# maxsonate/video-diffusion-nnx

Hardware: AMD Instinct MI355X
Metric: denoised frames/sec, 16fx64x64 1000-step DDPM (higher is better)
Workload: dtype bf16; 1 GPU; config_v2_2 (north-star shape): Unet3D dim=64 C=1, 16f x 64x64, DDPM T=1000 p_sample_loop (UNet forward + p_sample per step, hipGraph replay); value = n_gpus*B*F/(T*s_per_step); batch_per_gpu=64, parallelism=dp1 (independent samples, no collective), mfma_operands=bf16, storage=weights fp32 master, activations bf16, fp32 accumulate, process_group=none (single process)

## Files before the change

### video_diffusion_nnx_amd/csrc/conv_pw.hip

```cpp
#include "vdx_common.h"
#include "vdx_internal.h"

namespace vdx {

typedef unsigned pu32x4 __attribute__((ext_vector_type(4)));

template <int ROWS, int KS = 4, bool OUT32 = false>
__global__ __launch_bounds__(512) void conv1x1_pw_kernel(const ConvArgs P, const int nct, const int groups_per_range, const int ngroups) {
    using M = Mma<MODE_BF16>;
    constexpr int TM = ROWS / 16, TN = 2;
    constexpr int KBB = KS * 64;
    extern __shared__ __attribute__((aligned(16))) char smem[];
    const int Cin = P.C0 + P.C1, nkb = Cin / (32 * KS);
    const int WRS = Cin * 2 + 16;
    char* Wl = smem;
    float* bl = reinterpret_cast<float*>(Wl + ROWS * WRS);

    const int tid = threadIdx.x, lane = tid & 63, wave = tid >> 6, lp = lane & 15, q = lane >> 4;
    const int ct = (blockIdx.x >> 3) % nct, range = ((blockIdx.x >> 3) / nct) * 8 + (blockIdx.x & 7);
    const int co0 = ct * ROWS;
    const int g0 = range * groups_per_range, g1 = min(g0 + groups_per_range, ngroups);
    if (g0 >= g1) return;

    {
        const int cpr = Cin >> 3;
        const char* wsrc = reinterpret_cast<const char*>(P.wp);
        for (int i = tid; i < ROWS * cpr; i += 512) {
            const int row = i / cpr, c = i - row * cpr;
            const int tm = row >> 4, rr = row & 15;
            const int co = co0 + (tm >> 1) * 32 + (rr >> 2) * 8 + (tm & 1) * 4 + (rr & 3);
            *reinterpret_cast<uint4*>(Wl + row * WRS + c * 16) = *reinterpret_cast<const uint4*>(wsrc + ((size_t)(P.wrow0 + co) * P.CinPad + c * 8) * 2);
        }
        for (int i = tid; i < ROWS; i += 512) bl[i] = P.bias ? P.bias[co0 + i] : 0.f;
    }
    __syncthreads();

    const __amdgpu_buffer_rsrc_t rx0 = __builtin_amdgcn_make_buffer_rsrc(const_cast<float*>(P.x0), 0, P.x0_bytes, 0x00020000);
    const __amdgpu_buffer_rsrc_t rx1 = __builtin_amdgcn_make_buffer_rsrc(const_cast<float*>(P.C1 ? P.x1 : P.x0), 0, P.C1 ? P.x1_bytes : P.x0_bytes, 0x00020000);
    const int nkb0 = P.C0 / (32 * KS);
    const unsigned rb0 = P.C0 * 2, rb1 = P.C1 * 2;

    auto load_block = [&](int g, int kb, pu32x4 (&xf)[KS][TN]) {
        const bool second = kb >= nkb0;
        const unsigned rb = second ? rb1 : rb0;
        const unsigned base = (unsigned)(g * 32 + lp) * rb + (unsigned)((second ? kb - nkb0 : kb) * KBB + q * 16);
#pragma unroll
        for (int s = 0; s < KS; ++s)
#pragma unroll
            for (int tn = 0; tn < TN; ++tn) {
                const unsigned off = base + tn * 16 * rb + s * 64;
                xf[s][tn] = second ? __builtin_amdgcn_raw_buffer_load_b128(rx1, off, 0, 0) : __builtin_amdgcn_raw_buffer_load_b128(rx0, off, 0, 0);
            }
    };
    f32x4 acc[TM][TN];
    auto mma_block = [&](int kb, const pu32x4 (&xf)[KS][TN]) {
#pragma unroll
        for (int s = 0; s < KS; ++s) {
            uint4 bf[TN];
#pragma unroll
            for (int tn = 0; tn < TN; ++tn) bf[tn] = make_uint4(xf[s][tn].x, xf[s][tn].y, xf[s][tn].z, xf[s][tn].w);
#pragma unroll
            for (int tm = 0; tm < TM; ++tm) {
                const uint4 af = *reinterpret_cast<const uint4*>(Wl + (tm * 16 + lp) * WRS + kb * KBB + s * 64 + q * 16);
#pragma unroll
                for (int tn = 0; tn < TN; ++tn) M::mma(acc[tm][tn], af, bf[tn]);
            }
        }
    };

    char* const yb = reinterpret_cast<char*>(P.y);
    const char* const resb = reinterpret_cast<const char*>(P.res);
    constexpr bool PP = ROWS == 64 && KS == 4;
    auto init_acc = [&]() {
#pragma unroll
        for (int tm = 0; tm < TM; ++tm) {
            const float4 b4 = *reinterpret_cast<const float4*>(bl + (tm >> 1) * 32 + q * 8 + (tm & 1) * 4);
#pragma unroll
            for (int tn = 0; tn < TN; ++tn) acc[tm][tn] = f32x4{b4.x, b4.y, b4.z, b4.w};
        }
    };
    auto store_group = [&](int g) {
#pragma unroll
        for (int tn = 0; tn < TN; ++tn) {
            const size_t pix = (size_t)g * 32 + tn * 16 + lp;
#pragma unroll
            for (int j = 0; j < TM / 2; ++j) {
                const size_t el = pix * P.Cout + co0 + j * 32 + q * 8;
                float o[8];
#pragma unroll
                for (int k = 0; k < 4; ++k) { o[k] = acc[2 * j][tn][k]; o[4 + k] = acc[2 * j + 1][tn][k]; }
                if constexpr (OUT32) {
                    if (resb) {
                        const float4 r0 = *reinterpret_cast<const float4*>(resb + el * 4), r1 = *reinterpret_cast<const float4*>(resb + el * 4 + 16);
                        o[0] += r0.x; o[1] += r0.y; o[2] += r0.z; o[3] += r0.w; o[4] += r1.x; o[5] += r1.y; o[6] += r1.z; o[7] += r1.w;
                    }
                    *reinterpret_cast<float4*>(yb + el * 4) = make_float4(o[0], o[1], o[2], o[3]);
                    *reinterpret_cast<float4*>(yb + el * 4 + 16) = make_float4(o[4], o[5], o[6], o[7]);
                } else {
                    const size_t e = el * 2;
                    if (resb) {
                        const uint4 r = *reinterpret_cast<const uint4*>(resb + e);
                        o[0] += __uint_as_float(r.x << 16); o[1] += __uint_as_float(r.x & 0xFFFF0000u);
                        o[2] += __uint_as_float(r.y << 16); o[3] += __uint_as_float(r.y & 0xFFFF0000u);
                        o[4] += __uint_as_float(r.z << 16); o[5] += __uint_as_float(r.z & 0xFFFF0000u);
                        o[6] += __uint_as_float(r.w << 16); o[7] += __uint_as_float(r.w & 0xFFFF0000u);
                    }
                    *reinterpret_cast<uint4*>(yb + e) = make_uint4(pack_bf16x2(o[0], o[1]), pack_bf16x2(o[2], o[3]), pack_bf16x2(o[4], o[5]), pack_bf16x2(o[6], o[7]));
                }
            }
        }
    };
    if constexpr (KS == 2) {
        pu32x4 xa[KS][TN], xb[KS][TN];
        int g = g0 + wave;
        if (g < g1) load_block(g, 0, xa);
        for (; g < g1; g += 16) {
            __asm__ volatile("" ::: "memory");
            if (g + 8 < g1) load_block(g + 8, 0, xb);
            init_acc(); mma_block(0, xa); store_group(g);
            if (g + 8 >= g1) break;
            if (g + 16 < g1) load_block(g + 16, 0, xa);
            init_acc(); mma_block(0, xb); store_group(g + 8);
        }
    } else {
        pu32x4 xa[KS][TN], xb[PP ? KS : 1][TN];
        for (int g = g0 + wave; g < g1; g += 8) {
            __asm__ volatile("" ::: "memory");
            init_acc();
            load_block(g, 0, xa);
            if constexpr (PP) {
                for (int kb = 0; kb < nkb; kb += 2) {
                    if (kb + 1 < nkb) load_block(g, kb + 1, xb);
                    mma_block(kb, xa);
                    if (kb + 1 >= nkb) break;
                    if (kb + 2 < nkb) load_block(g, kb + 2, xa);
                    mma_block(kb + 1, xb);
                }
            } else {
                for (int kb = 0; kb < nkb; ++kb) {
                    mma_block(kb, xa);
                    if (kb + 1 < nkb) load_block(g, kb + 1, xa);
                }
            }
            store_group(g);
        }
    }
}

int conv1x1_pw_rows(const ConvArgs& a) {
    const int cin = a.C0 + a.C1;
    if (a.Cout % 128 == 0 && (size_t)128 * (cin * 2 + 16) + 128 * 4 <= 140 * 1024) return 128;
    return 64;
}

bool conv1x1_pw_eligible(int mode, const ConvArgs& a) {
    if (mode != MODE_BF16 || a.kind != 0 || a.kh != 1 || a.kw != 1 || a.stride != 1 || a.pad != 0 || a.pro || a.out_stats) return false;
    if (!a.x0_bf16 || (a.C1 && !a.x1_bf16)) return false;
    const bool out32 = !a.y_bf16;
    if (a.res && (a.res_bf16 != 0) == out32) return false;
    const int cin = a.C0 + a.C1;
    if ((cin % 128 && cin != 64) || cin > 1024 || a.Cout % 64 || a.Cout < 64) return false;
    if (out32 && cin == 64) return false;
    if (!out32 && cin != 64 && a.Cout < 128) return false;
    if (a.C1 && (a.C0 % 128 || a.C1 % 128)) return false;
    if (a.CinPad != cin) return false;
    const size_t npix = (size_t)a.NF * a.H * a.W;
    if (npix % 32 || npix < 32 * 256) return false;
    if (npix * (size_t)std::max(std::max(a.C0, a.C1), a.Cout) * 2 >= 0xFFFF0000ull) return false;
    const int rows = conv1x1_pw_rows(a);
    if ((size_t)rows * (cin * 2 + 16) + rows * 4 > 160 * 1024) return false;
    return true;
}

hipError_t launch_conv1x1_pw(const ConvArgs& a, hipStream_t st) {
    const int cin = a.C0 + a.C1, rows = conv1x1_pw_rows(a), nct = a.Cout / rows;
    const int ngroups = (int)((size_t)a.NF * a.H * a.W / 32);
    const int cus = device_cus();
    const size_t lds = (size_t)rows * (cin * 2 + 16) + rows * 4;
    const int wg_per_cu = (lds <= 80 * 1024 && rows == 128) ? 2 : 1;
    int nranges = std::max(8, (cus * wg_per_cu / nct) / 8 * 8);
    int gpr = ((ngroups + nranges - 1) / nranges + 7) / 8 * 8;
    nranges = ((ngroups + gpr - 1) / gpr + 7) / 8 * 8;
    auto go = [&](auto kfn) -> hipError_t {
        if (hipError_t e = lds_opt_in(kfn, lds); e != hipSuccess) return e;
        hipLaunchKernelGGL(kfn, dim3(nranges * nct), dim3(512), lds, st, a, nct, gpr, ngroups);
        return hipGetLastError();
    };
    if (!a.y_bf16) return rows == 128 ? go(conv1x1_pw_kernel<128, 4, true>) : go(conv1x1_pw_kernel<64, 4, true>);
    if (cin == 64) return rows == 128 ? go(conv1x1_pw_kernel<128, 2>) : go(conv1x1_pw_kernel<64, 2>);
    return rows == 128 ? go(conv1x1_pw_kernel<128>) : go(conv1x1_pw_kernel<64>);
}

}
```

### video_diffusion_nnx_amd/csrc/elementwise.hip

```cpp
#include "vdx_common.h"
#include <stdlib.h>
#include "vdx_internal.h"

namespace vdx {

template <int VPL>
__global__ __launch_bounds__(256) void resblock_tail_kernel(TailArgs P) {
    __shared__ float coefA[1024], coefD[1024];
    __shared__ float gm[64];
    const int tid = threadIdx.x;
    const int C = P.C;
    const int b = blockIdx.y;
    gn_mean_rstd_wg(P.stats, b, P.groups, (double)P.pix_per_sample * (C / P.groups), gm, tid, 256);
    __syncthreads();
    for (int c = tid; c < C; c += 256) {
        const int g = c / (C / P.groups);
        const float a = gm[2 * g + 1] * P.gn_gamma[c];
        coefA[c] = a;
        coefD[c] = P.gn_beta[c] - gm[2 * g] * a;
    }
    __syncthreads();
    const int LPP = P.lpp;
    const int ppb = 256 / LPP;
    const int sub = tid % LPP, pl = tid / LPP;
    const float invC = 1.0f / (float)C;
    for (long pix = (long)blockIdx.x * ppb + pl; pix < P.pix_per_sample; pix += (long)gridDim.x * ppb) {
        const size_t base = ((size_t)b * P.pix_per_sample + pix) * C;
        float4 r[VPL];
        float s = 0.f, ss = 0.f;
#pragma unroll
        for (int v = 0; v < VPL; ++v) {
            const int c = (v * LPP + sub) * 4;
            r[v] = make_float4(0.f, 0.f, 0.f, 0.f);
            if (c < C) {
                r[v] = load4_f32_or_bf16(P.r, base + c, P.r_bf16);
                s += r[v].x + r[v].y + r[v].z + r[v].w;
                ss += r[v].x * r[v].x + r[v].y * r[v].y + r[v].z * r[v].z + r[v].w * r[v].w;
            }
        }
        for (int o = 1; o < LPP; o <<= 1) { s += __shfl_xor(s, o); ss += __shfl_xor(ss, o); }
        const float mean = s * invC;
        const float var = fmaxf(ss * invC - mean * mean, 0.f);
        const float rstd = rsqrtf(var + NORM_EPS);
#pragma unroll
        for (int v = 0; v < VPL; ++v) {
            const int c = (v * LPP + sub) * 4;
            if (c < C) {
                const float4 y = load4_f32_or_bf16(P.y2, base + c, P.y2_bf16);
                const float4 a = *reinterpret_cast<const float4*>(coefA + c);
                const float4 d = *reinterpret_cast<const float4*>(coefD + c);
                const float4 lg = *reinterpret_cast<const float4*>(P.ln_gamma + c);
                const float4 lb = *reinterpret_cast<const float4*>(P.ln_beta + c);
                float4 o;
                o.x = silu_f(fmaf(y.x, a.x, d.x)) + fmaf((r[v].x - mean) * rstd, lg.x, lb.x);
                o.y = silu_f(fmaf(y.y, a.y, d.y)) + fmaf((r[v].y - mean) * rstd, lg.y, lb.y);
                o.z = silu_f(fmaf(y.z, a.z, d.z)) + fmaf((r[v].z - mean) * rstd, lg.z, lb.z);
                o.w = silu_f(fmaf(y.w, a.w, d.w)) + fmaf((r[v].w - mean) * rstd, lg.w, lb.w);
                store4_f32_or_bf16(P.out, base + c, o, P.out_bf16);
            }
        }
    }
}

__device__ __forceinline__ void unpack8(const uint4& u, float (&f)[8]) {
    f[0] = __uint_as_float(u.x << 16); f[1] = __uint_as_float(u.x & 0xFFFF0000u);
    f[2] = __uint_as_float(u.y << 16); f[3] = __uint_as_float(u.y & 0xFFFF0000u);
    f[4] = __uint_as_float(u.z << 16); f[5] = __uint_as_float(u.z & 0xFFFF0000u);
    f[6] = __uint_as_float(u.w << 16); f[7] = __uint_as_float(u.w & 0xFFFF0000u);
}

template <int VPL>
__global__ __launch_bounds__(256) void resblock_tail16_kernel(TailArgs P) {
    __shared__ float coefA[1024], coefD[1024];
    __shared__ float gm[64];
    const int tid = threadIdx.x;
    const int C = P.C;
    const int b = blockIdx.y;
    gn_mean_rstd_wg(P.stats, b, P.groups, (double)P.pix_per_sample * (C / P.groups), gm, tid, 256);
    __syncthreads();
    for (int c = tid; c < C; c += 256) {
        const int g = c / (C / P.groups);
        const float a = gm[2 * g + 1] * P.gn_gamma[c];
        coefA[c] = a;
        coefD[c] = P.gn_beta[c] - gm[2 * g] * a;
    }
    __syncthreads();
    const int LPP = P.lpp;
    const int ppb = 256 / LPP;
    const int sub = tid % LPP, pl = tid / LPP;
    const float invC = 1.0f / (float)C;
    const char* rb = reinterpret_cast<const char*>(P.r);
    const char* yb = reinterpret_cast<const char*>(P.y2);
    char* ob = reinterpret_cast<char*>(P.out);
    for (long pix = (long)blockIdx.x * ppb + pl; pix < P.pix_per_sample; pix += (long)gridDim.x * ppb) {
        const size_t base = ((size_t)b * P.pix_per_sample + pix) * C;
        float r[VPL][8];
        float s = 0.f, ss = 0.f;
#pragma unroll
        for (int v = 0; v < VPL; ++v) {
            const int c = (v * LPP + sub) * 8;
#pragma unroll
            for (int k = 0; k < 8; ++k) r[v][k] = 0.f;
            if (c < C) {
                unpack8(*reinterpret_cast<const uint4*>(rb + (base + c) * 2), r[v]);
#pragma unroll
                for (int k = 0; k < 8; ++k) { s += r[v][k]; ss += r[v][k] * r[v][k]; }
            }
        }
        for (int o = 1; o < LPP; o <<= 1) { s += __shfl_xor(s, o); ss += __shfl_xor(ss, o); }
        const float mean = s * invC;
        const float var = fmaxf(ss * invC - mean * mean, 0.f);
        const float rstd = rsqrtf(var + NORM_EPS);
#pragma unroll
        for (int v = 0; v < VPL; ++v) {
            const int c = (v * LPP + sub) * 8;
            if (c < C) {
                float y[8], o[8];
                unpack8(*reinterpret_cast<const uint4*>(yb + (base + c) * 2), y);
#pragma unroll
                for (int k = 0; k < 8; ++k)
                    o[k] = silu_f(fmaf(y[k], coefA[c + k], coefD[c + k])) + fmaf((r[v][k] - mean) * rstd, P.ln_gamma[c + k], P.ln_beta[c + k]);
                *reinterpret_cast<uint4*>(ob + (base + c) * 2) =
                    make_uint4(pack_bf16x2(o[0], o[1]), pack_bf16x2(o[2], o[3]), pack_bf16x2(o[4], o[5]), pack_bf16x2(o[6], o[7]));
            }
        }
    }
}

__global__ __launch_bounds__(256) void gn_silu_apply16_kernel(unsigned* __restrict__ y, const double* __restrict__ stats, const float* __restrict__ gamma,
                                                              const float* __restrict__ beta, const float* __restrict__ ss, int ss_stride, int groups,
                                                              int C, long pix_per_sample) {
    __shared__ float coefA[1024], coefD[1024];
    __shared__ float gm[64];
    const int tid = threadIdx.x, b = blockIdx.y;
    gn_mean_rstd_wg(stats, b, groups, (double)pix_per_sample * (C / groups), gm, tid, 256);
    __syncthreads();
    for (int c = tid; c < C; c += 256) {
        const int g = c / (C / groups);
        const float m = gm[2 * g], rs = gm[2 * g + 1];
        const float ga = gamma[c], be = beta[c];
        float sc = 1.f, sh = 0.f;
        if (ss) { sc = ss[(size_t)b * ss_stride + c] + 1.f; sh = ss[(size_t)b * ss_stride + C + c]; }
        coefA[c] = rs * ga * sc;
        coefD[c] = (be - m * rs * ga) * sc + sh;
    }
    __syncthreads();
    const int octs = C >> 3;
    const long n = pix_per_sample * octs;
    uint4* base = reinterpret_cast<uint4*>(y) + (size_t)b * n;
    for (long i0 = (long)blockIdx.x * 1024 + tid; i0 < n; i0 += (long)gridDim.x * 1024) {
        uint4 v[4];
#pragma unroll
        for (int u = 0; u < 4; ++u) v[u] = (i0 + u * 256 < n) ? base[i0 + u * 256] : make_uint4(0u, 0u, 0u, 0u);
#pragma unroll
        for (int u = 0; u < 4; ++u) {
            if (i0 + u * 256 >= n) continue;
            const int c = (int)((i0 + u * 256) % octs) * 8;
            float f[8], o[8];
            unpack8(v[u], f);
#pragma unroll
            for (int k = 0; k < 8; ++k) o[k] = silu_f(fmaf(f[k], coefA[c + k], coefD[c + k]));
            base[i0 + u * 256] = make_uint4(pack_bf16x2(o[0], o[1]), pack_bf16x2(o[2], o[3]), pack_bf16x2(o[4], o[5]), pack_bf16x2(o[6], o[7]));
        }
    }
}

hipError_t launch_gn_silu_apply16(float* y_bf16, const double* stats, const float* gamma, const float* beta, const float* ss, int ss_stride, int groups,
                                  int C, int batch, long pix_per_sample, hipStream_t st) {
    if (C % 8 || C > 1024 || groups <= 0 || groups > 32 || C % groups) return hipErrorInvalidValue;
    const long n = pix_per_sample * (C / 8);
    const int gx = (int)std::max<long>(1, std::min<long>((n + 1023) / 1024, 2048));
    LaunchScope ls(st, "gn_silu_apply16_kernel", 8.0 * batch * pix_per_sample * C, 4.0 * batch * pix_per_sample * C, "C%d px%ld x %d", C, pix_per_sample, batch);
    hipLaunchKernelGGL(gn_silu_apply16_kernel, dim3(gx, batch), dim3(256), 0, st, reinterpret_cast<unsigned*>(y_bf16), stats, gamma, beta, ss, ss_stride, groups, C, pix_per_sample);
    return hipGetLastError();
}

typedef unsigned tu32x4 __attribute__((ext_vector_type(4)));

template <int CIN, int COUT, bool CAT, bool FIN = false>
__global__ __launch_bounds__(256, (CIN == 128 && COUT == 64) ? 4 : (COUT <= 128 ? 3 : 2)) void resblock_tail_rc16_kernel(TailArgs P) {
    using M = Mma<MODE_BF16>;
    constexpr int NTM = COUT / 16, NKS = CIN / 32, NH = COUT / 32;
    constexpr int C0 = CAT ? CIN / 2 : CIN, NK0 = C0 / 32;
    constexpr int WRS = CIN * 2 + 16;
    extern __shared__ __attribute__((aligned(16))) char smem[];
    char* Wl = smem;
    float* coefA = reinterpret_cast<float*>(Wl + COUT * WRS);
    float* coefD = coefA + COUT;
    float* lng = coefD + COUT;
    float* lnb = lng + COUT;
    float* rcb = lnb + COUT;
    float* gm = rcb + COUT;
    float* finw = gm + 64;
    const int tid = threadIdx.x, lane = tid & 63, wave = tid >> 6, lp = lane & 15, q = lane >> 4;
    const int b = blockIdx.y;
    for (int i = tid; i < COUT * (CIN / 8); i += 256) {
        const int row = i / (CIN / 8), c = i % (CIN / 8);
        const int tm = row >> 4, rr = row & 15;
        const int co = (tm >> 1) * 32 + (rr >> 2) * 8 + (tm & 1) * 4 + (rr & 3);
        *reinterpret_cast<uint4*>(Wl + row * WRS + c * 16) =
            *reinterpret_cast<const uint4*>(reinterpret_cast<const char*>(P.rc_w) + ((size_t)co * ((CIN + 63) / 64 * 64) + c * 8) * 2);
    }
    gn_mean_rstd_wg(P.stats, b, P.groups, (double)P.pix_per_sample * (COUT / P.groups), gm, tid, 256);
    __syncthreads();
    for (int c = tid; c < COUT; c += 256) {
        const int g = c / (COUT / P.groups);
        const float a = gm[2 * g + 1] * P.gn_gamma[c];
        coefA[c] = a;
        coefD[c] = P.gn_beta[c] - gm[2 * g] * a;
        lng[c] = P.ln_gamma[c]; lnb[c] = P.ln_beta[c]; rcb[c] = P.rc_b[c];
        if (FIN) finw[c] = P.fin_w[c];
    }
    __syncthreads();

    const unsigned pps = (unsigned)P.pix_per_sample;
    const char* x0p = reinterpret_cast<const char*>(P.x0) + (size_t)b * pps * C0 * 2;
    const char* x1p = CAT ? reinterpret_cast<const char*>(P.x1) + (size_t)b * pps * C0 * 2 : x0p;
    const char* y2p = reinterpret_cast<const char*>(P.y2) + (size_t)b * pps * COUT * 2;
    char* outp = FIN ? const_cast<char*>(y2p) : reinterpret_cast<char*>(P.out) + (size_t)b * pps * COUT * 2;
    float* const finp = FIN ? P.fin_out + (size_t)b * pps : nullptr;
    const float finb = FIN ? P.fin_b[0] : 0.f;
    const __amdgpu_buffer_rsrc_t rx0 = __builtin_amdgcn_make_buffer_rsrc(const_cast<char*>(x0p), 0, pps * C0 * 2, 0x00020000);
    const __amdgpu_buffer_rsrc_t rx1 = __builtin_amdgcn_make_buffer_rsrc(const_cast<char*>(x1p), 0, pps * C0 * 2, 0x00020000);
    const __amdgpu_buffer_rsrc_t ry = __builtin_amdgcn_make_buffer_rsrc(const_cast<char*>(y2p), 0, pps * COUT * 2, 0x00020000);
    const __amdgpu_buffer_rsrc_t ro = __builtin_amdgcn_make_buffer_rsrc(outp, 0, pps * COUT * 2, 0x00020000);
    const int ngroups = (int)(pps >> 4);
    const int gstride = (int)gridDim.x * 4;
    const unsigned lane_x = lp * (C0 * 2) + q * 16, lane_y = lp * (COUT * 2) + q * 16;

    auto issue = [&](int g, tu32x4 (&xf)[NKS], tu32x4 (&yf)[NH]) {
        const unsigned ox = (unsigned)g * (16 * C0 * 2) + lane_x, oy = (unsigned)g * (16 * COUT * 2) + lane_y;
#pragma unroll
        for (int s = 0; s < NKS; ++s)
            xf[s] = (s < NK0) ? __builtin_amdgcn_raw_buffer_load_b128(rx0, ox + s * 64, 0, 0)
                              : __builtin_amdgcn_raw_buffer_load_b128(rx1, ox + (s - NK0) * 64, 0, 0);
#pragma unroll
        for (int j = 0; j < NH; ++j) yf[j] = __builtin_amdgcn_raw_buffer_load_b128(ry, oy + j * 64, 0, 0);
    };
    auto compute = [&](int g, const tu32x4 (&xf)[NKS], const tu32x4 (&yf)[NH]) {
        __asm__ volatile("" ::: "memory");
        f32x4 acc[NTM];
#pragma unroll
        for (int tm = 0; tm < NTM; ++tm) {
            const float4 b4 = *reinterpret_cast<const float4*>(rcb + (tm >> 1) * 32 + q * 8 + (tm & 1) * 4);
            acc[tm] = f32x4{b4.x, b4.y, b4.z, b4.w};
        }
#pragma unroll
        for (int s = 0; s < NKS; ++s) {
            const uint4 bx = make_uint4(xf[s].x, xf[s].y, xf[s].z, xf[s].w);
#pragma unroll
            for (int tm = 0; tm < NTM; ++tm)
                M::mma(acc[tm], *reinterpret_cast<const uint4*>(Wl + (tm * 16 + lp) * WRS + s * 64 + q * 16), bx);
        }
        float s1 = 0.f, s2 = 0.f;
#pragma unroll
        for (int tm = 0; tm < NTM; ++tm)
#pragma unroll
            for (int e = 0; e < 4; ++e) { s1 += acc[tm][e]; s2 += acc[tm][e] * acc[tm][e]; }
        s1 = reduce_q(s1); s2 = reduce_q(s2);
        const float mean = s1 * (1.0f / COUT);
        const float var = fmaxf(s2 * (1.0f / COUT) - mean * mean, 0.f);
        const float rstd = rsqrtf(var + NORM_EPS);
        const unsigned oy = (unsigned)g * (16 * COUT * 2) + lane_y;
        float dot = 0.f;
#pragma unroll
        for (int j = 0; j < NH; ++j) {
            float y[8], o[8];
            unpack8(make_uint4(yf[j].x, yf[j].y, yf[j].z, yf[j].w), y);
            const int c0 = j * 32 + q * 8;
#pragma unroll
            for (int h = 0; h < 2; ++h) {
                const float4 a4 = *reinterpret_cast<const float4*>(coefA + c0 + 4 * h), d4 = *reinterpret_cast<const float4*>(coefD + c0 + 4 * h);
                const float4 g4 = *reinterpret_cast<const float4*>(lng + c0 + 4 * h), e4 = *reinterpret_cast<const float4*>(lnb + c0 + 4 * h);
                const f32x4 r = acc[2 * j + h];
                o[4 * h + 0] = silu_f(fmaf(y[4 * h + 0], a4.x, d4.x)) + fmaf((r[0] - mean) * rstd, g4.x, e4.x);
                o[4 * h + 1] = silu_f(fmaf(y[4 * h + 1], a4.y, d4.y)) + fmaf((r[1] - mean) * rstd, g4.y, e4.y);
                o[4 * h + 2] = silu_f(fmaf(y[4 * h + 2], a4.z, d4.z)) + fmaf((r[2] - mean) * rstd, g4.z, e4.z);
                o[4 * h + 3] = silu_f(fmaf(y[4 * h + 3], a4.w, d4.w)) + fmaf((r[3] - mean) * rstd, g4.w, e4.w);
            }
            if constexpr (FIN) {
                const float4 w0 = *reinterpret_cast<const float4*>(finw + c0), w1 = *reinterpret_cast<const float4*>(finw + c0 + 4);
                dot = fmaf(o[0], w0.x, dot); dot = fmaf(o[1], w0.y, dot); dot = fmaf(o[2], w0.z, dot); dot = fmaf(o[3], w0.w, dot);
                dot = fmaf(o[4], w1.x, dot); dot = fmaf(o[5], w1.y, dot); dot = fmaf(o[6], w1.z, dot); dot = fmaf(o[7], w1.w, dot);
            } else {
                __builtin_amdgcn_raw_buffer_store_b128(tu32x4{pack_bf16x2(o[0], o[1]), pack_bf16x2(o[2], o[3]), pack_bf16x2(o[4], o[5]), pack_bf16x2(o[6], o[7])},
                                                       ro, oy + j * 64, 0, 0);
            }
        }
        if constexpr (FIN) {
            dot = reduce_q(dot);
            if (q == 0) finp[(size_t)g * 16 + lp] = dot + finb;
        }
    };

    tu32x4 xa[NKS], ya[NH], xb[NKS], yb[NH];
    int g = (int)blockIdx.x * 4 + wave;
    if (g < ngroups) issue(g, xa, ya);
    while (g < ngroups) {
        const int g1 = g + gstride;
        if (g1 < ngroups) issue(g1, xb, yb);
        compute(g, xa, ya);
        if (g1 >= ngroups) break;
        g = g1 + gstride;
        if (g < ngroups) issue(g, xa, ya);
        compute(g1, xb, yb);
    }
}

bool tail_rc16_supported(int cin, int c0, int cout, long pix_per_sample) {
    const bool shape = (cin == 128 && cout == 64) || (cin == 64 && cout == 128) || (cin == 256 && cout == 64) || (cin == 128 && cout == 256) ||
                       (cin == 64 && cout == 32) || (cin == 32 && cout == 64) || (cin == 128 && cout == 32);
    return shape && (c0 == cin || 2 * c0 == cin) && pix_per_sample % 16 == 0 && pix_per_sample * std::max(cin, cout) * 2 < (1L << 31);
}

template <int CIN, int COUT>
static hipError_t launch_tail_rc16(const TailArgs& a, hipStream_t st) {
    const size_t lds = (size_t)COUT * (CIN * 2 + 16) + (6 * COUT + 64) * sizeof(float);
    const long need = (a.pix_per_sample / 16 + 3) / 4;
    const long gx = std::min<long>(need, std::max<long>(std::max<long>(1, need / 8), (2048 + a.batch - 1) / std::max(1, a.batch)));
    auto go = [&](auto kfn) -> hipError_t {
        if (hipError_t e = lds_opt_in(kfn, lds); e != hipSuccess) return e;
        const double px = (double)a.batch * a.pix_per_sample;
        LaunchScope ls(st, "resblock_tail_rc16_kernel", 2.0 * px * CIN * COUT + (a.fin_w ? 2.0 * px * COUT : 0.0),
                       px * (CIN + (a.fin_w ? 1.0 : 2.0) * COUT) * 2 + (a.fin_w ? px * 4 : 0.0) + 2.0 * CIN * COUT, "<%d, %d, %s> px%ld x %d", CIN, COUT,
                       a.fin_w ? "true, head" : (a.C1 ? "true" : "false"), a.pix_per_sample, a.batch);
        hipLaunchKernelGGL(kfn, dim3((unsigned)gx, a.batch), dim3(256), lds, st, a);
        return hipGetLastError();
    };
    if constexpr ((CIN == 128 && COUT == 64) || (CIN == 64 && COUT == 32)) {
        if (a.fin_w) return a.C1 ? go(resblock_tail_rc16_kernel<CIN, COUT, true, true>) : hipErrorInvalidValue;
    } else if (a.fin_w) return hipErrorInvalidValue;
    return a.C1 ? go(resblock_tail_rc16_kernel<CIN, COUT, true>) : go(resblock_tail_rc16_kernel<CIN, COUT, false>);
}

hipError_t launch_resblock_tail(TailArgs a, hipStream_t st) {
    if (a.rc_w) {
        const int cin = a.C0 + a.C1;
        if (!(a.y2_bf16 && a.out_bf16) || !a.x0 || (a.C1 && !a.x1) || !a.rc_b || !tail_rc16_supported(cin, a.C0, a.C, a.pix_per_sample))
            return hipErrorInvalidValue;
        if (a.groups <= 0 || a.groups > 32 || a.C % a.groups) return hipErrorInvalidValue;
        if (cin == 128 && a.C == 64) return launch_tail_rc16<128, 64>(a, st);
        if (cin == 64 && a.C == 128) return launch_tail_rc16<64, 128>(a, st);
        if (cin == 256 && a.C == 64) return launch_tail_rc16<256, 64>(a, st);
        if (cin == 64 && a.C == 32) return launch_tail_rc16<64, 32>(a, st);
        if (cin == 32 && a.C == 64) return launch_tail_rc16<32, 64>(a, st);
        if (cin == 128 && a.C == 32) return launch_tail_rc16<128, 32>(a, st);
        return launch_tail_rc16<128, 256>(a, st);
    }
    if (a.y2_bf16 && a.r_bf16 && a.out_bf16 && a.C % 8 == 0) {
        const int octs = a.C / 8;
        int lpp = 1;
        while (lpp < octs && lpp < 64) lpp <<= 1;
        a.lpp = lpp;
        const int vpl = (octs + lpp - 1) / lpp;
        const int ppb = 256 / lpp;
        const int tail_wgs = 0;
        const long need = (a.pix_per_sample + ppb - 1) / ppb;
        const long total = tail_wgs > 0 ? tail_wgs : std::max<long>(2048, need * a.batch / 8);
        const int gx = (int)std::min<long>(need, std::max<long>(1, std::min<long>(2048, total / std::max(1, a.batch))));
        dim3 grid(gx, a.batch);
        const double el = (double)a.batch * a.pix_per_sample * a.C;
        LaunchScope ls(st, "resblock_tail16_kernel", 10.0 * el, 3.0 * el * 2, "<%d> C%d px%ld x %d", vpl, a.C, a.pix_per_sample, a.batch);
        switch (vpl) {
            case 1: hipLaunchKernelGGL(resblock_tail16_kernel<1>, grid, dim3(256), 0, st, a); break;
            case 2: hipLaunchKernelGGL(resblock_tail16_kernel<2>, grid, dim3(256), 0, st, a); break;
            default: return hipErrorInvalidValue;
        }
        return hipGetLastError();
    }
    const int quads = a.C / 4;
    int lpp = 1;
    while (lpp < quads && lpp < 64) lpp <<= 1;
    a.lpp = lpp;
    const int vpl = (quads + lpp - 1) / lpp;
    const int ppb = 256 / lpp;
    const int tail_wgs32 = 0;
    const long need32 = (a.pix_per_sample + ppb - 1) / ppb;
    const long total32 = tail_wgs32 > 0 ? tail_wgs32 : std::max<long>(2048, need32 * a.batch / 8);
    int gx = (int)std::min<long>(need32, std::max<long>(1, std::min<long>(2048, total32 / std::max(1, a.batch))));
    dim3 grid(gx, a.batch);
    const double el = (double)a.batch * a.pix_per_sample * a.C;
    LaunchScope ls(st, "resblock_tail_kernel", 10.0 * el, el * ((a.y2_bf16 ? 2.0 : 4.0) + (a.r_bf16 ? 2.0 : 4.0) + (a.out_bf16 ? 2.0 : 4.0)), "<%d> C%d px%ld x %d y2_16 %d", vpl == 3 ? 4 : vpl,
                   a.C, a.pix_per_sample, a.batch, a.y2_bf16);
    switch (vpl) {
        case 1: hipLaunchKernelGGL(resblock_tail_kernel<1>, grid, dim3(256), 0, st, a); break;
        case 2: hipLaunchKernelGGL(resblock_tail_kernel<2>, grid, dim3(256), 0, st, a); break;
        case 3: case 4: hipLaunchKernelGGL(resblock_tail_kernel<4>, grid, dim3(256), 0, st, a); break;
        default: return hipErrorInvalidValue;
    }
    return hipGetLastError();
}

__global__ __launch_bounds__(256) void init_conv_kernel(const float* __restrict__ x, const float* __restrict__ w,
                                                        const float* __restrict__ bias, float* __restrict__ y,
                                                        int B, int Cin, int F, int H, int W, int Cout, int K, int y_bf16) {
    extern __shared__ float tile[];
    const int pad = K / 2, TW = 16 + K - 1;
    const int tx = blockIdx.x % ((W + 15) / 16), ty = blockIdx.x / ((W + 15) / 16);
    const int f = blockIdx.y % F, b = blockIdx.y / F;
    const int cg = blockIdx.z;
    for (int i = threadIdx.x; i < Cin * TW * TW; i += 256) {
        const int c = i / (TW * TW), r = i % (TW * TW);
        const int gy = ty * 16 + r / TW - pad, gx = tx * 16 + r % TW - pad;
        float v = 0.f;
        if (gy >= 0 && gy < H && gx >= 0 && gx < W) v = x[((((size_t)b * Cin + c) * F + f) * H + gy) * W + gx];
        tile[i] = v;
    }
    __syncthreads();
    const int px = threadIdx.x & 15, py = threadIdx.x >> 4;
    float acc[16];
#pragma unroll
    for (int j = 0; j < 16; ++j) acc[j] = 0.f;
    const int co0 = cg * 16;
    for (int c = 0; c < Cin; ++c)
        for (int ky = 0; ky < K; ++ky)
            for (int kx = 0; kx < K; ++kx) {
                const float v = tile[(c * TW + py + ky) * TW + px + kx];
                const float* wr = w + ((size_t)(ky * K + kx) * Cin + c) * Cout + co0;
#pragma unroll
                for (int j = 0; j < 16; ++j) acc[j] = fmaf(v, (co0 + j < Cout) ? wr[j] : 0.f, acc[j]);
            }
    const int oy = ty * 16 + py, ox = tx * 16 + px;
    if (oy < H && ox < W) {
        const size_t ob = ((((size_t)b * F + f) * H + oy) * W + ox) * Cout + co0;
        if (co0 + 16 <= Cout) {
#pragma unroll
            for (int j = 0; j < 16; j += 4)
                store4_f32_or_bf16(y, ob + j, make_float4(acc[j] + bias[co0 + j], acc[j + 1] + bias[co0 + j + 1],
                                                          acc[j + 2] + bias[co0 + j + 2], acc[j + 3] + bias[co0 + j + 3]), y_bf16);
        } else {
            for (int j = 0; j < 16 && co0 + j < Cout; ++j) {
                if (y_bf16) reinterpret_cast<__bf16*>(y)[ob + j] = (__bf16)(acc[j] + bias[co0 + j]);
                else y[ob + j] = acc[j] + bias[co0 + j];
            }
        }
    }
}

__global__ __launch_bounds__(256) void init_conv_mfma_kernel(const float* __restrict__ x, const float* __restrict__ w,
                                                             const float* __restrict__ bias, float* __restrict__ y,
                                                             int B, int F, int H, int W, int Cout, int K, int y_bf16) {
    using M = Mma<MODE_BF16>;
    constexpr int KP = 64, RSK = KP * 2 + 16;
    constexpr int TWM = 16 + 8 - 1;
    extern __shared__ __attribute__((aligned(16))) char smem[];
    float* tile = reinterpret_cast<float*>(smem);
    char* wl = smem + ((TWM * TWM * 4 + 15) / 16) * 16;
    char* col = wl + 64 * RSK;
    const int tid = threadIdx.x, lane = tid & 63, wv = tid >> 6;
    const int lp = lane & 15, q = lane >> 4;
    const int pad = K / 2, TW = 16 + K - 1;
    const int tx = blockIdx.x % ((W + 15) / 16), ty = blockIdx.x / ((W + 15) / 16);
    const int f = blockIdx.y % F, b = blockIdx.y / F;
    for (int i = tid; i < TW * TW; i += 256) {
        const int gy = ty * 16 + i / TW - pad, gx = tx * 16 + i % TW - pad;
        tile[i] = (gy >= 0 && gy < H && gx >= 0 && gx < W) ? x[(((size_t)b * F + f) * H + gy) * W + gx] : 0.f;
    }
    for (int i = tid; i < 64 * RSK / 4; i += 256) reinterpret_cast<unsigned*>(wl)[i] = 0u;
    __syncthreads();
    {
        float wr[16];
        const int nw = K * K * Cout;
#pragma unroll
        for (int u = 0; u < 16; ++u) { const int i = tid + u * 256; wr[u] = w[i < nw ? i : 0]; }
#pragma unroll
        for (int u = 0; u < 16; ++u) {
            const int i = tid + u * 256;
            if (i < nw) {
                const int co = i % Cout, t = i / Cout;
                if (co < 64) M::store1(wl + co * RSK, (t / K) * 8 + (t % K), wr[u]);
            }
        }
    }
    {
        const int py = tid >> 4, px = tid & 15;
        char* row = col + tid * RSK;
#pragma unroll
        for (int ky = 0; ky < 8; ++ky) {
            float v[8];
#pragma unroll
            for (int kx = 0; kx < 8; ++kx) v[kx] = (ky < K && kx < K) ? tile[(py + ky) * TW + px + kx] : 0.f;
            *reinterpret_cast<uint4*>(row + ky * 16) =
                make_uint4(pack_bf16x2(v[0], v[1]), pack_bf16x2(v[2], v[3]), pack_bf16x2(v[4], v[5]), pack_bf16x2(v[6], v[7]));
        }
    }
    __syncthreads();
    f32x4 acc[4][4];
#pragma unroll
    for (int i = 0; i < 4; ++i)
#pragma unroll
        for (int j = 0; j < 4; ++j) acc[i][j] = f32x4{0.f, 0.f, 0.f, 0.f};
#pragma unroll
    for (int ch = 0; ch < 2; ++ch) {
        uint4 af[4], bf[4];
#pragma unroll
        for (int tm = 0; tm < 4; ++tm) af[tm] = *reinterpret_cast<const uint4*>(wl + (tm * 16 + lp) * RSK + ch * 64 + q * 16);
#pragma unroll
        for (int tn = 0; tn < 4; ++tn) bf[tn] = *reinterpret_cast<const uint4*>(col + ((wv * 4 + tn) * 16 + lp) * RSK + ch * 64 + q * 16);
#pragma unroll
        for (int tm = 0; tm < 4; ++tm)
#pragma unroll
            for (int tn = 0; tn < 4; ++tn) M::mma(acc[tm][tn], af[tm], bf[tn]);
    }
    if (y_bf16 && Cout == 64) {
        __syncthreads();
#pragma unroll
        for (int tn = 0; tn < 4; ++tn)
#pragma unroll
            for (int tm = 0; tm < 4; ++tm) {
                const float4 bi = *reinterpret_cast<const float4*>(bias + tm * 16 + 4 * q);
                *reinterpret_cast<uint2*>(col + ((wv * 4 + tn) * 16 + lp) * RSK + (tm * 16 + 4 * q) * 2) =
                    make_uint2(pack_bf16x2(acc[tm][tn][0] + bi.x, acc[tm][tn][1] + bi.y), pack_bf16x2(acc[tm][tn][2] + bi.z, acc[tm][tn][3] + bi.w));
            }
        __syncthreads();
#pragma unroll
        for (int u = 0; u < 8; ++u) {
            const int i = tid + u * 256, p = i >> 3, pc = i & 7;
            const int oy = ty * 16 + (p >> 4), ox = tx * 16 + (p & 15);
            if (oy < H && ox < W)
                *reinterpret_cast<uint4*>(reinterpret_cast<char*>(y) + (((((size_t)b * F + f) * H + oy) * W + ox) * 64) * 2 + pc * 16) =
                    *reinterpret_cast<const uint4*>(col + p * RSK + pc * 16);
        }
        return;
    }
#pragma unroll
    for (int tn = 0; tn < 4; ++tn) {
        const int p = (wv * 4 + tn) * 16 + lp;
        const int oy = ty * 16 + (p >> 4), ox = tx * 16 + (p & 15);
        if (oy >= H || ox >= W) continue;
        const size_t ob = ((((size_t)b * F + f) * H + oy) * W + ox) * Cout;
#pragma unroll
        for (int tm = 0; tm < 4; ++tm) {
            const int co = tm * 16 + 4 * q;
            if (co >= Cout) continue;
            const float4 bi = *reinterpret_cast<const float4*>(bias + co);
            store4_f32_or_bf16(y, ob + co, make_float4(acc[tm][tn][0] + bi.x, acc[tm][tn][1] + bi.y, acc[tm][tn][2] + bi.z, acc[tm][tn][3] + bi.w), y_bf16);
        }
    }
}

hipError_t launch_init_conv(const float* x, const float* w, const float* bias, float* y, int B, int Cin, int F, int H, int W,
                            int Cout, int K, int y_bf16, hipStream_t st) {
    return launch_init_conv_mode(MODE_F32, x, w, bias, y, B, Cin, F, H, W, Cout, K, y_bf16, st);
}

hipError_t launch_init_conv_mode(int mode, const float* x, const float* w, const float* bias, float* y, int B, int Cin, int F, int H, int W,
                                 int Cout, int K, int y_bf16, hipStream_t st) {
    if (mode == MODE_BF16 && Cin == 1 && K <= 8 && Cout <= 64 && Cout % 4 == 0) {
        const size_t lds = ((23 * 23 * 4 + 15) / 16) * 16 + (size_t)(64 + 256) * (64 * 2 + 16);
        dim3 grid(((W + 15) / 16) * ((H + 15) / 16), B * F);
        const double px = (double)B * F * H * W;
        LaunchScope ls(st, "init_conv_mfma_kernel", 2.0 * px * K * K * Cout, px * (4.0 + Cout * (y_bf16 ? 2.0 : 4.0)), "k%d 1->%d %dx%dx%d", K, Cout, B * F, H, W);
        hipLaunchKernelGGL(init_conv_mfma_kernel, grid, dim3(256), lds, st, x, w, bias, y, B, F, H, W, Cout, K, y_bf16);
        return hipGetLastError();
    }
    const int TW = 16 + K - 1;
    dim3 grid(((W + 15) / 16) * ((H + 15) / 16), B * F, (Cout + 15) / 16);
    const double px = (double)B * F * H * W;
    LaunchScope ls(st, "init_conv_kernel", 2.0 * px * K * K * Cin * Cout, px * (4.0 * Cin + Cout * (y_bf16 ? 2.0 : 4.0)), "k%d %d->%d %dx%dx%d", K, Cin, Cout, B * F, H, W);
    hipLaunchKernelGGL(init_conv_kernel, grid, dim3(256), (size_t)Cin * TW * TW * 4, st, x, w, bias, y, B, Cin, F, H, W, Cout, K, y_bf16);
    return hipGetLastError();
}

__global__ __launch_bounds__(256) void final_conv_kernel(const float* __restrict__ x, const float* __restrict__ w,
                                                         const float* __restrict__ bias, float* __restrict__ y,
                                                         long npix, int D, int Cout, int lpp, int x_bf16) {
    const int sub = threadIdx.x % lpp, pl = threadIdx.x / lpp, ppb = 256 / lpp;
    for (long pix = (long)blockIdx.x * ppb + pl; pix < npix; pix += (long)gridDim.x * ppb) {
        for (int co = 0; co < Cout; ++co) {
            float s = 0.f;
            if (x_bf16) {
                for (int c = sub * 8; c < D; c += lpp * 8) {
                    float v[8];
                    unpack8(*reinterpret_cast<const uint4*>(reinterpret_cast<const char*>(x) + ((size_t)pix * D + c) * 2), v);
#pragma unroll
                    for (int k = 0; k < 8; ++k) s = fmaf(v[k], w[(size_t)(c + k) * Cout + co], s);
                }
            } else {
                for (int c = sub * 4; c < D; c += lpp * 4) {
                    const float4 v = *reinterpret_cast<const float4*>(x + (size_t)pix * D + c);
                    s += v.x * w[(size_t)c * Cout + co] + v.y * w[(size_t)(c + 1) * Cout + co]
                       + v.z * w[(size_t)(c + 2) * Cout + co] + v.w * w[(size_t)(c + 3) * Cout + co];
                }
            }
            for (int o = 1; o < lpp; o <<= 1) s += __shfl_xor(s, o);
            if (sub == 0) y[(size_t)pix * Cout + co] = s + bias[co];
        }
    }
}

template <int COUT>
__global__ __launch_bounds__(256) void final_conv16_kernel(const float* __restrict__ x, const float* __restrict__ w,
                                                           const float* __restrict__ bias, float* __restrict__ y, long npix, int D, int lpp) {
    constexpr int U = 4;
    const int sub = threadIdx.x % lpp, pl = threadIdx.x / lpp, ppb = 256 / lpp;
    float wr[COUT][8], br[COUT];
#pragma unroll
    for (int co = 0; co < COUT; ++co) {
        br[co] = bias[co];
#pragma unroll
        for (int k = 0; k < 8; ++k) wr[co][k] = w[(size_t)(sub * 8 + k) * COUT + co];
    }
    for (long g0 = (long)blockIdx.x * U; g0 * ppb < npix; g0 += (long)gridDim.x * U) {
        uint4 raw[U];
#pragma unroll
        for (int u = 0; u < U; ++u) {
            const long pix = (g0 + u) * ppb + pl;
            raw[u] = *reinterpret_cast<const uint4*>(reinterpret_cast<const char*>(x) + ((size_t)(pix < npix ? pix : 0) * D + sub * 8) * 2);
        }
#pragma unroll
        for (int u = 0; u < U; ++u) {
            const long pix = (g0 + u) * ppb + pl;
            float v[8];
            unpack8(raw[u], v);
#pragma unroll
            for (int co = 0; co < COUT; ++co) {
                float s = 0.f;
#pragma unroll
                for (int k = 0; k < 8; ++k) s = fmaf(v[k], wr[co][k], s);
                for (int o = 1; o < lpp; o <<= 1) s += __shfl_xor(s, o);
                if (sub == 0 && pix < npix) y[(size_t)pix * COUT + co] = s + br[co];
            }
        }
    }
}

hipError_t launch_final_conv(const float* x, const float* w, const float* bias, float* y, long npix, int D, int Cout, int x_bf16, hipStream_t st) {
    if (x_bf16 && D % 8 == 0 && D <= 128 && ((D / 8) & (D / 8 - 1)) == 0 && Cout >= 1 && Cout <= 4) {
        const int lpp = D / 8, ppb = 256 / lpp;
        const int blocks = (int)std::min<long>((npix + 4L * ppb - 1) / (4L * ppb), 4096);
        LaunchScope ls(st, "final_conv16_kernel", 2.0 * npix * D * Cout, (double)npix * (D * 2.0 + Cout * 4.0), "<%d> D%d px%ld", Cout, D, npix);
        switch (Cout) {
            case 1: hipLaunchKernelGGL(final_conv16_kernel<1>, dim3(blocks), dim3(256), 0, st, x, w, bias, y, npix, D, lpp); break;
            case 2: hipLaunchKernelGGL(final_conv16_kernel<2>, dim3(blocks), dim3(256), 0, st, x, w, bias, y, npix, D, lpp); break;
            case 3: hipLaunchKernelGGL(final_conv16_kernel<3>, dim3(blocks), dim3(256), 0, st, x, w, bias, y, npix, D, lpp); break;
            default: hipLaunchKernelGGL(final_conv16_kernel<4>, dim3(blocks), dim3(256), 0, st, x, w, bias, y, npix, D, lpp); break;
        }
        return hipGetLastError();
    }
    const int per = (x_bf16 && D % 8 == 0) ? 8 : 4;
    if (per == 4) x_bf16 = x_bf16 ? -1 : 0;
    if (x_bf16 < 0) return hipErrorInvalidValue;
    int lpp = 1;
    while (lpp * per < D && lpp < 16) lpp <<= 1;
    const int ppb = 256 / lpp;
    const int blocks = (int)std::min<long>((npix + ppb - 1) / ppb, 4096);
    LaunchScope ls(st, "final_conv_kernel", 2.0 * npix * D * Cout, (double)npix * (D * (x_bf16 ? 2.0 : 4.0) + Cout * 4.0), "D%d->%d px%ld", D, Cout, npix);
    hipLaunchKernelGGL(final_conv_kernel, dim3(blocks), dim3(256), 0, st, x, w, bias, y, npix, D, Cout, lpp, x_bf16);
    return hipGetLastError();
}

__device__ __forceinline__ float gelu_tanh_f(float x) {
    return 0.5f * x * (1.0f + tanhf(0.7978845608028654f * (x + 0.044715f * x * x * x)));
}

__global__ __launch_bounds__(256) void time_mlp_kernel(TimeMlpArgs P) {
    extern __shared__ float sm[];
    float* emb = sm;
    float* h = sm + P.dim;
    const int b = blockIdx.x, tid = threadIdx.x;
    const int half = P.dim / 2;
    const float tval = P.t_is_device_scalar ? (float)P.time[0] : (float)P.time[b];
    for (int i = tid; i < half; i += 256) {
        const float fr = expf((float)i * -(logf(10000.0f) / (float)(half - 1)));
        const float arg = tval * fr;
        emb[i] = sinf(arg);
        emb[half + i] = cosf(arg);
    }
    __syncthreads();
    for (int n = tid; n < P.time_dim; n += 256) {
        float a0 = P.b1[n], a1 = 0.f, a2 = 0.f, a3 = 0.f;
// ... 122 lines not shown
```

Before: 48.67 frames/s.

## Swizzle pointwise-conv LDS weights, pipeline loads across groups, and unroll resblock tail

The 1x1 conv kernel drops the LDS row padding in favour of an XOR swizzle, batches the weight staging loads, and issues the first input and residual loads before weight staging. In the KS=4 bf16-output case it adds a continuous two-stage pipeline across groups with residual prefetch. The resblock tail kernel is templated on lanes-per-pixel, uses DPP/permlane reductions, caches coefficients in registers and processes four pixels per iteration with batched loads. It also changes launch sizing and occupancy for both kernels. Register pressure rises, and the swizzle must exactly match the MFMA read pattern.

```diff
diff --git a/video_diffusion_nnx_amd/csrc/conv_pw.hip b/video_diffusion_nnx_amd/csrc/conv_pw.hip
--- a/video_diffusion_nnx_amd/csrc/conv_pw.hip
+++ b/video_diffusion_nnx_amd/csrc/conv_pw.hip
@@ -12,28 +12,40 @@
     constexpr int KBB = KS * 64;
     extern __shared__ __attribute__((aligned(16))) char smem[];
     const int Cin = P.C0 + P.C1, nkb = Cin / (32 * KS);
-    const int WRS = Cin * 2 + 16;
+    const int WRS = Cin * 2;
     char* Wl = smem;
     float* bl = reinterpret_cast<float*>(Wl + ROWS * WRS);
 
-    const int tid = threadIdx.x, lane = tid & 63, wave = tid >> 6, lp = lane & 15, q = lane >> 4;
+    const int tid = threadIdx.x, lane = tid & 63, lp = lane & 15, q = lane >> 4;
+    const int wave = __builtin_amdgcn_readfirstlane(tid >> 6);
     const int ct = (blockIdx.x >> 3) % nct, range = ((blockIdx.x >> 3) / nct) * 8 + (blockIdx.x & 7);
     const int co0 = ct * ROWS;
     const int g0 = range * groups_per_range, g1 = min(g0 + groups_per_range, ngroups);
     if (g0 >= g1) return;
 
-    {
+    auto stage_weights = [&]() {
         const int cpr = Cin >> 3;
         const char* wsrc = reinterpret_cast<const char*>(P.wp);
-        for (int i = tid; i < ROWS * cpr; i += 512) {
-            const int row = i / cpr, c = i - row * cpr;
-            const int tm = row >> 4, rr = row & 15;
-            const int co = co0 + (tm >> 1) * 32 + (rr >> 2) * 8 + (tm & 1) * 4 + (rr & 3);
-            *reinterpret_cast<uint4*>(Wl + row * WRS + c * 16) = *reinterpret_cast<const uint4*>(wsrc + ((size_t)(P.wrow0 + co) * P.CinPad + c * 8) * 2);
+        constexpr int WB = 8;
+        for (int i0 = tid; i0 < ROWS * cpr; i0 += 512 * WB) {
+            uint4 wv[WB];
+            int dst[WB];
+#pragma unroll
+            for (int u = 0; u < WB; ++u) {
+                const int i = min(i0 + u * 512, ROWS * cpr - 1);
+                const int row = i / cpr, c = i - row * cpr;
+                const int tm = row >> 4, rr = row & 15;
+                const int co = co0 + (tm >> 1) * 32 + (rr >> 2) * 8 + (tm & 1) * 4 + (rr & 3);
+                dst[u] = row * WRS + ((c ^ (KS == 2 ? (rr >> 1) & 7 : rr)) << 4);
+                wv[u] = *reinterpret_cast<const uint4*>(wsrc + ((size_t)(P.wrow0 + co) * P.CinPad + c * 8) * 2);
+            }
+#pragma unroll
+            for (int u = 0; u < WB; ++u)
+                *reinterpret_cast<uint4*>(Wl + dst[u]) = wv[u];
         }
         for (int i = tid; i < ROWS; i += 512) bl[i] = P.bias ? P.bias[co0 + i] : 0.f;
-    }
-    __syncthreads();
+        __syncthreads();
+    };
 
     const __amdgpu_buffer_rsrc_t rx0 = __builtin_amdgcn_make_buffer_rsrc(const_cast<float*>(P.x0), 0, P.x0_bytes, 0x00020000);
     const __amdgpu_buffer_rsrc_t rx1 = __builtin_amdgcn_make_buffer_rsrc(const_cast<float*>(P.C1 ? P.x1 : P.x0), 0, P.C1 ? P.x1_bytes : P.x0_bytes, 0x00020000);
@@ -52,6 +64,7 @@
                 xf[s][tn] = second ? __builtin_amdgcn_raw_buffer_load_b128(rx1, off, 0, 0) : __builtin_amdgcn_raw_buffer_load_b128(rx0, off, 0, 0);
             }
     };
+    const int swz = (KS == 2 ? (lp >> 1) & 7 : lp) << 4;
     f32x4 acc[TM][TN];
     auto mma_block = [&](int kb, const pu32x4 (&xf)[KS][TN]) {
 #pragma unroll
@@ -61,7 +74,7 @@
             for (int tn = 0; tn < TN; ++tn) bf[tn] = make_uint4(xf[s][tn].x, xf[s][tn].y, xf[s][tn].z, xf[s][tn].w);
 #pragma unroll
             for (int tm = 0; tm < TM; ++tm) {
-                const uint4 af = *reinterpret_cast<const uint4*>(Wl + (tm * 16 + lp) * WRS + kb * KBB + s * 64 + q * 16);
+                const uint4 af = *reinterpret_cast<const uint4*>(Wl + (tm * 16 + lp) * WRS + ((kb * KBB + s * 64 + q * 16) ^ swz));
 #pragma unroll
                 for (int tn = 0; tn < TN; ++tn) M::mma(acc[tm][tn], af, bf[tn]);
             }
@@ -78,6 +91,15 @@
 #pragma unroll
             for (int tn = 0; tn < TN; ++tn) acc[tm][tn] = f32x4{b4.x, b4.y, b4.z, b4.w};
         }
+    };
+    constexpr bool PIPE = KS == 4 && !OUT32;
+    pu32x4 rf[TM / 2][TN];
+    auto load_res = [&](int g) {
+#pragma unroll
+        for (int tn = 0; tn < TN; ++tn)
+#pragma unroll
+            for (int j = 0; j < TM / 2; ++j)
+                rf[j][tn] = *reinterpret_cast<const pu32x4*>(resb + (((size_t)g * 32 + tn * 16 + lp) * P.Cout + co0 + j * 32 + q * 8) * 2);
     };
     auto store_group = [&](int g) {
 #pragma unroll
@@ -99,7 +121,7 @@
                 } else {
                     const size_t e = el * 2;
                     if (resb) {
-                        const uint4 r = *reinterpret_cast<const uint4*>(resb + e);
+                        const uint4 r = PIPE ? make_uint4(rf[j][tn].x, rf[j][tn].y, rf[j][tn].z, rf[j][tn].w) : *reinterpret_cast<const uint4*>(resb + e);
                         o[0] += __uint_as_float(r.x << 16); o[1] += __uint_as_float(r.x & 0xFFFF0000u);
                         o[2] += __uint_as_float(r.y << 16); o[3] += __uint_as_float(r.y & 0xFFFF0000u);
                         o[4] += __uint_as_float(r.z << 16); o[5] += __uint_as_float(r.z & 0xFFFF0000u);
@@ -110,7 +132,37 @@
             }
         }
     };
-    if constexpr (KS == 2) {
+    if constexpr (PIPE) {
+        constexpr int NS = 2;
+        pu32x4 xs[NS][KS][TN];
+        auto adv = [&](int& gg, int& kk) { if (++kk == nkb) { kk = 0; gg += 8; } };
+        int g = g0 + wave, kb = 0;
+        int pg = g, pk = 0;
+#pragma unroll
+        for (int i = 0; i < NS - 1; ++i) {
+            if (pg < g1) load_block(pg, pk, xs[i]);
+            adv(pg, pk);
+        }
+        if (resb && g < g1) load_res(g);
+        stage_weights();
+        while (g < g1) {
+#pragma unroll
+            for (int i = 0; i < NS; ++i) {
+                if (g >= g1) break;
+                __asm__ volatile("" ::: "memory");
+                if (pg < g1) load_block(pg, pk, xs[(i + NS - 1) % NS]);
+                adv(pg, pk);
+                if (kb == 0) init_acc();
+                mma_block(kb, xs[i]);
+                if (kb == nkb - 1) {
+                    store_group(g);
+                    if (resb && g + 8 < g1) load_res(g + 8);
+                }
+                adv(g, kb);
+            }
+        }
+    } else if constexpr (KS == 2) {
+        stage_weights();
         pu32x4 xa[KS][TN], xb[KS][TN];
         int g = g0 + wave;
         if (g < g1) load_block(g, 0, xa);
@@ -123,6 +175,7 @@
             init_acc(); mma_block(0, xb); store_group(g + 8);
         }
     } else {
+        stage_weights();
         pu32x4 xa[KS][TN], xb[PP ? KS : 1][TN];
         for (int g = g0 + wave; g < g1; g += 8) {
             __asm__ volatile("" ::: "memory");
@@ -149,7 +202,7 @@
 
 int conv1x1_pw_rows(const ConvArgs& a) {
     const int cin = a.C0 + a.C1;
-    if (a.Cout % 128 == 0 && (size_t)128 * (cin * 2 + 16) + 128 * 4 <= 140 * 1024) return 128;
+    if (a.Cout % 128 == 0 && (size_t)128 * (cin * 2) + 128 * 4 <= 140 * 1024) return 128;
     return 64;
 }
 
@@ -168,7 +221,7 @@
     if (npix % 32 || npix < 32 * 256) return false;
     if (npix * (size_t)std::max(std::max(a.C0, a.C1), a.Cout) * 2 >= 0xFFFF0000ull) return false;
     const int rows = conv1x1_pw_rows(a);
-    if ((size_t)rows * (cin * 2 + 16) + rows * 4 > 160 * 1024) return false;
+    if ((size_t)rows * (cin * 2) + rows * 4 > 160 * 1024) return false;
     return true;
 }
 
@@ -176,8 +229,8 @@
     const int cin = a.C0 + a.C1, rows = conv1x1_pw_rows(a), nct = a.Cout / rows;
     const int ngroups = (int)((size_t)a.NF * a.H * a.W / 32);
     const int cus = device_cus();
-    const size_t lds = (size_t)rows * (cin * 2 + 16) + rows * 4;
-    const int wg_per_cu = (lds <= 80 * 1024 && rows == 128) ? 2 : 1;
+    const size_t lds = (size_t)rows * (cin * 2) + rows * 4;
+    const int wg_per_cu = (lds <= 80 * 1024 && rows == 128 && (!a.y_bf16 || cin == 64)) ? 2 : 1;
     int nranges = std::max(8, (cus * wg_per_cu / nct) / 8 * 8);
     int gpr = ((ngroups + nranges - 1) / nranges + 7) / 8 * 8;
     nranges = ((ngroups + gpr - 1) / gpr + 7) / 8 * 8;
diff --git a/video_diffusion_nnx_amd/csrc/elementwise.hip b/video_diffusion_nnx_amd/csrc/elementwise.hip
--- a/video_diffusion_nnx_amd/csrc/elementwise.hip
+++ b/video_diffusion_nnx_amd/csrc/elementwise.hip
@@ -69,7 +69,25 @@
     f[6] = __uint_as_float(u.w << 16); f[7] = __uint_as_float(u.w & 0xFFFF0000u);
 }
 
-template <int VPL>
+template <int LPP>
+__device__ __forceinline__ float reduce_lpp(float v) {
+    if constexpr (LPP > 1) v += dpp_row<0xB1>(v);
+    if constexpr (LPP > 2) v += dpp_row<0x4E>(v);
+    if constexpr (LPP > 4) v += dpp_row<0x141>(v);
+    if constexpr (LPP > 8) v += dpp_row<0x140>(v);
+    if constexpr (LPP > 16) {
+        const auto t = __builtin_amdgcn_permlane16_swap(__float_as_uint(v), __float_as_uint(v), false, false);
+        v = __uint_as_float(t[0]) + __uint_as_float(t[1]);
+    }
+    if constexpr (LPP > 32) {
+        const auto t = __builtin_amdgcn_permlane32_swap(__float_as_uint(v), __float_as_uint(v), false, false);
+        v = __uint_as_float(t[0]) + __uint_as_float(t[1]);
+    }
+    return v;
+}
+
+constexpr int TAIL_U = 4;
+template <int VPL, int LPP>
 __global__ __launch_bounds__(256) void resblock_tail16_kernel(TailArgs P) {
     __shared__ float coefA[1024], coefD[1024];
     __shared__ float gm[64];
@@ -85,43 +103,73 @@
         coefD[c] = P.gn_beta[c] - gm[2 * g] * a;
     }
     __syncthreads();
-    const int LPP = P.lpp;
-    const int ppb = 256 / LPP;
+    constexpr int ppb = 256 / LPP;
     const int sub = tid % LPP, pl = tid / LPP;
     const float invC = 1.0f / (float)C;
-    const char* rb = reinterpret_cast<const char*>(P.r);
-    const char* yb = reinterpret_cast<const char*>(P.y2);
-    char* ob = reinterpret_cast<char*>(P.out);
-    for (long pix = (long)blockIdx.x * ppb + pl; pix < P.pix_per_sample; pix += (long)gridDim.x * ppb) {
-        const size_t base = ((size_t)b * P.pix_per_sample + pix) * C;
-        float r[VPL][8];
-        float s = 0.f, ss = 0.f;
-#pragma unroll
-        for (int v = 0; v < VPL; ++v) {
-            const int c = (v * LPP + sub) * 8;
-#pragma unroll
-            for (int k = 0; k < 8; ++k) r[v][k] = 0.f;
-            if (c < C) {
-                unpack8(*reinterpret_cast<const uint4*>(rb + (base + c) * 2), r[v]);
+    float cA[VPL][8], cD[VPL][8], lg[VPL][8], lb[VPL][8];
+    bool cv[VPL];
+    unsigned cb[VPL];
+#pragma unroll
+    for (int v = 0; v < VPL; ++v) {
+        const int c = (v * LPP + sub) * 8;
+        cv[v] = c < C;
+        const int cc = cv[v] ? c : 0;
+        cb[v] = (unsigned)cc * 2;
+#pragma unroll
+        for (int h = 0; h < 2; ++h) {
+            const float4 a4 = *reinterpret_cast<const float4*>(coefA + cc + 4 * h), d4 = *reinterpret_cast<const float4*>(coefD + cc + 4 * h);
+            cA[v][4 * h] = a4.x; cA[v][4 * h + 1] = a4.y; cA[v][4 * h + 2] = a4.z; cA[v][4 * h + 3] = a4.w;
+            cD[v][4 * h] = d4.x; cD[v][4 * h + 1] = d4.y; cD[v][4 * h + 2] = d4.z; cD[v][4 * h + 3] = d4.w;
+        }
+#pragma unroll
+        for (int k = 0; k < 8; ++k) { lg[v][k] = P.ln_gamma[cc + k]; lb[v][k] = P.ln_beta[cc + k]; }
+    }
+    const long pps = P.pix_per_sample;
+    const size_t rowb = (size_t)C * 2;
+    const char* __restrict__ rb = reinterpret_cast<const char*>(P.r) + (size_t)b * pps * rowb;
+    const char* __restrict__ yb = reinterpret_cast<const char*>(P.y2) + (size_t)b * pps * rowb;
+    char* __restrict__ ob = reinterpret_cast<char*>(P.out) + (size_t)b * pps * rowb;
+    for (long p0 = (long)blockIdx.x * (TAIL_U * ppb); p0 < pps; p0 += (long)gridDim.x * (TAIL_U * ppb)) {
+        uint4 rr[TAIL_U][VPL], yy[TAIL_U][VPL];
+#pragma unroll
+        for (int u = 0; u < TAIL_U; ++u) {
+            const long pix = p0 + u * ppb + pl;
+            const size_t base = (size_t)(pix < pps ? pix : 0) * rowb;
+#pragma unroll
+            for (int v = 0; v < VPL; ++v) rr[u][v] = *reinterpret_cast<const uint4*>(rb + base + cb[v]);
+        }
+#pragma unroll
+        for (int u = 0; u < TAIL_U; ++u) {
+            const long pix = p0 + u * ppb + pl;
+            const size_t base = (size_t)(pix < pps ? pix : 0) * rowb;
+#pragma unroll
+            for (int v = 0; v < VPL; ++v) yy[u][v] = *reinterpret_cast<const uint4*>(yb + base + cb[v]);
+        }
+#pragma unroll
+        for (int u = 0; u < TAIL_U; ++u) {
+            const long pix = p0 + u * ppb + pl;
+            float r[VPL][8];
+            float s = 0.f, ss = 0.f;
+#pragma unroll
+            for (int v = 0; v < VPL; ++v) {
+                unpack8(cv[v] ? rr[u][v] : make_uint4(0u, 0u, 0u, 0u), r[v]);
 #pragma unroll
                 for (int k = 0; k < 8; ++k) { s += r[v][k]; ss += r[v][k] * r[v][k]; }
             }
-        }
-        for (int o = 1; o < LPP; o <<= 1) { s += __shfl_xor(s, o); ss += __shfl_xor(ss, o); }
-        const float mean = s * invC;
-        const float var = fmaxf(ss * invC - mean * mean, 0.f);
-        const float rstd = rsqrtf(var + NORM_EPS);
-#pragma unroll
-        for (int v = 0; v < VPL; ++v) {
-            const int c = (v * LPP + sub) * 8;
-            if (c < C) {
+            s = reduce_lpp<LPP>(s); ss = reduce_lpp<LPP>(ss);
+            const float mean = s * invC;
+            const float var = fmaxf(ss * invC - mean * mean, 0.f);
+            const float rstd = rsqrtf(var + NORM_EPS);
+#pragma unroll
+            for (int v = 0; v < VPL; ++v) {
                 float y[8], o[8];
-                unpack8(*reinterpret_cast<const uint4*>(yb + (base + c) * 2), y);
+                unpack8(yy[u][v], y);
 #pragma unroll
                 for (int k = 0; k < 8; ++k)
-                    o[k] = silu_f(fmaf(y[k], coefA[c + k], coefD[c + k])) + fmaf((r[v][k] - mean) * rstd, P.ln_gamma[c + k], P.ln_beta[c + k]);
-                *reinterpret_cast<uint4*>(ob + (base + c) * 2) =
-                    make_uint4(pack_bf16x2(o[0], o[1]), pack_bf16x2(o[2], o[3]), pack_bf16x2(o[4], o[5]), pack_bf16x2(o[6], o[7]));
+                    o[k] = silu_f(fmaf(y[k], cA[v][k], cD[v][k])) + fmaf((r[v][k] - mean) * rstd, lg[v][k], lb[v][k]);
+                if (pix < pps && cv[v])
+                    *reinterpret_cast<uint4*>(ob + (size_t)pix * rowb + cb[v]) =
+                        make_uint4(pack_bf16x2(o[0], o[1]), pack_bf16x2(o[2], o[3]), pack_bf16x2(o[4], o[5]), pack_bf16x2(o[6], o[7]));
             }
         }
     }
@@ -354,19 +402,26 @@
         a.lpp = lpp;
         const int vpl = (octs + lpp - 1) / lpp;
         const int ppb = 256 / lpp;
-        const int tail_wgs = 0;
-        const long need = (a.pix_per_sample + ppb - 1) / ppb;
-        const long total = tail_wgs > 0 ? tail_wgs : std::max<long>(2048, need * a.batch / 8);
-        const int gx = (int)std::min<long>(need, std::max<long>(1, std::min<long>(2048, total / std::max(1, a.batch))));
+        const long need = (a.pix_per_sample + TAIL_U * ppb - 1) / (TAIL_U * ppb);
+        const int gx = (int)std::max<long>(1, std::min<long>(need, 1024));
         dim3 grid(gx, a.batch);
         const double el = (double)a.batch * a.pix_per_sample * a.C;
         LaunchScope ls(st, "resblock_tail16_kernel", 10.0 * el, 3.0 * el * 2, "<%d> C%d px%ld x %d", vpl, a.C, a.pix_per_sample, a.batch);
-        switch (vpl) {
-            case 1: hipLaunchKernelGGL(resblock_tail16_kernel<1>, grid, dim3(256), 0, st, a); break;
-            case 2: hipLaunchKernelGGL(resblock_tail16_kernel<2>, grid, dim3(256), 0, st, a); break;
-            default: return hipErrorInvalidValue;
-        }
-        return hipGetLastError();
+        auto go = [&](auto kfn) -> hipError_t {
+            hipLaunchKernelGGL(kfn, grid, dim3(256), 0, st, a);
+            return hipGetLastError();
+        };
+        if (vpl == 2) return go(resblock_tail16_kernel<2, 64>);
+        if (vpl != 1) return hipErrorInvalidValue;
+        switch (lpp) {
+            case 1: return go(resblock_tail16_kernel<1, 1>);
+            case 2: return go(resblock_tail16_kernel<1, 2>);
+            case 4: return go(resblock_tail16_kernel<1, 4>);
+            case 8: return go(resblock_tail16_kernel<1, 8>);
+            case 16: return go(resblock_tail16_kernel<1, 16>);
+            case 32: return go(resblock_tail16_kernel<1, 32>);
+            default: return go(resblock_tail16_kernel<1, 64>);
+        }
     }
     const int quads = a.C / 4;
     int lpp = 1;
```

Result: no change. 48.98 frames/s (median of 6 runs) (+0.6%).
